# alexklwong/calibrated-backprojection-network

Hardware: AMD Instinct MI355X
Metric: depth-completion frames/sec at 352x1216 (higher is better)
Workload: dtype f32; 1 GPU; KITTI 352x1216, batch 32/GPU, fp32, full KBNet forward in HIP, random xavier weights; frames_per_gpu=32, global_batch=32, height=352, width=1216, n_ranks_seen=1, collective_backend=nccl, gathered_frames=32, launch=HIP graph replay, 2 concurrent sub-batch branch(es)

## Files before the change

calibrated-backprojection-network_amd/_lib.py:

```python

from __future__ import annotations

import ctypes as C
import os

import torch

HERE = os.path.dirname(os.path.abspath(__file__))
LIB_PATH = os.environ.get("KBN_LIB_PATH") or os.path.join(HERE, "libkbnet_hip.so")

KBN_OK = 0
KBN_ERR_INVALID_ARGUMENT, KBN_ERR_UNSUPPORTED, KBN_ERR_WORKSPACE, KBN_ERR_LAUNCH = -1, -2, -3, -4
KBN_SRC_TENSOR, KBN_SRC_COORDS, KBN_SRC_XYZ, KBN_SRC_PAIR = 0, 1, 2, 3
KBN_ACT_ELU, KBN_ACT_SIGMOID = 1, 2
KBN_RESIZE_NONE, KBN_RESIZE_NEAREST = 0, 1
KBN_MAX_SRC = 3
ABI_VERSION = 7


class KbnError(RuntimeError):
    pass


class ConvSrc(C.Structure):
    _fields_ = [
        ("kind", C.c_int),
        ("channels", C.c_int),
        ("data", C.c_void_p),
        ("batch_stride", C.c_longlong),
        ("src_height", C.c_int),
        ("src_width", C.c_int),
        ("aux_channels", C.c_int),
# ... 58 lines not shown
    "kbn_depth_head_forward": (_I, [_P, _P, _P, _P, _I, _I, _I, _I, _F, _F, _P]),
    "kbn_conv_head_forward": (_I, [_P, _L, _P, _P, _P, _P, _I, _I, _I, _I, _I, _F, _F, _F, _P]),
    "kbn_conv_tail_packed_weight_bytes": (C.c_size_t, [_I]),
    "kbn_conv_tail_pack_weight": (_I, [_P, _P, _I, _P]),
    "kbn_conv_tail_forward": (_I, [_P, _L, _P, _P, _P, _P, _I, _I, _I, _I, _I, _F, _F, _F, _P]),
    "kbn_conv_tail_forward_pair": (_I, [_P, _L, _P, _P, _P, _P, _P, _I, _I, _I, _I, _I, _F, _F, _F, _P]),
    "kbn_absmax_frames": (_I, [_P, _L, _I, _L, _P, _P]),
    "kbn_conv3x3_split_packed_weight_bytes": (C.c_size_t, [_I, _I, _I]),
    "kbn_conv3x3_split_pack_weight": (_I, [_P, _P, _I, _I, _I, _P]),
    "kbn_conv3x3_split_forward": (_I, [C.POINTER(ConvSrc), _I, _P, _P, _L, _I, _I, _I, _I, _I, _I, _I, _F, _P, _P, _L, _P, _P]),
    "kbn_conv3x3_split_forward_ksplit": (_I, [C.POINTER(ConvSrc), _I, _P, _P, _L, _I, _I, _I, _I, _I, _I, _I, _F, _P, _I, _P, _P]),
    "kbn_conv1x1s2_split_packed_weight_bytes": (C.c_size_t, [_I, _I, _I]),
    "kbn_conv1x1s2_split_pack_weight": (_I, [_P, _P, _I, _I, _I, _P]),
    "kbn_conv1x1s2_split_forward": (_I, [C.POINTER(ConvSrc), _I, _P, _P, _L, _P, _L, _I, _I, _I, _I, _I, _I, _F, _P, _P]),
    "kbn_kb_xyz_s2_forward": (_I, [_P, _L, _I, _I, _I, _P, _P, _I, _F, _P, _L, _I, _P]),
    "kbn_png_info": (_I, [_P, C.c_size_t, _P, _P, _P, _P]),
    "kbn_png_decode": (_I, [_P, C.c_size_t, _P, C.c_size_t]),
    "kbn_png_decode_batch": (_I, [_P, _P, _P, _P, _I, _I, _P]),
    "kbn_depth_to_u16_forward": (_I, [_P, _P, _L, _P]),
    "kbn_png_encode_gray16_bound": (C.c_size_t, [_I, _I]),
    "kbn_png_encode_gray16": (_I, [_P, _I, _I, _P, C.c_size_t, _P, _I]),
    "kbn_unpack_frames_forward": (_I, [_P, _P, _P, _P, _I, _I, _I, _I, _I, _I, _I, _P]),
}

_lib = None


def load():
    global _lib
    if _lib is not None:
# ... 31 lines not shown
```

calibrated-backprojection-network_amd/csrc/abi.hip:

```cpp
#include <stdlib.h>
#include <string.h>

#include "kbn_common.h"

namespace kbn {

KnobValue g_knobs[KNOB_COUNT];

static const char* const kKnobNames[KNOB_COUNT] = {
    "KBN_DEBUG", "KBN_FORCE_MW", "KBN_FORCE_TWB", "KBN_EPI_LDS", "KBN_NO_WINO",
    "KBN_NO_UP2X9", "KBN_NO_UP2X3", "KBN_WINO_RT",
    "KBN_NO_KB_PAIR", "KBN_NO_KB_DEPTH_FUSION", "KBN_PAIR_CAND", "KBN_S2D_DEBUG", "KBN_AUTOTUNE",
    "KBN_NO_HEAD_FUSION", "KBN_NO_SPLIT", "KBN_NO_OVERLAP", "KBN_NO_PAIR", "KBN_NO_PAIR_MID", "KBN_NO_PAIR_ENC",
    "KBN_NO_PAIR_TAIL", "KBN_NO_DEPTH_FRONT_FUSION", "KBN_FP16_ONE_TERM", "KBN_DEPTH_FRONT_FUSION", "KBN_NO_FRONT_NEXT"};

void tune_reload_env();

static void load_knobs() {
    for (int k = 0; k < KNOB_COUNT; ++k) {
        const char* v = getenv(kKnobNames[k]);
        g_knobs[k].set = (v && *v) ? 1 : 0;
        int val = 0;
        if (v && *v) {
            char* end = nullptr;
            const long parsed = strtol(v, &end, 10);
            val = (end == v) ? 1 : (int)parsed;
        }
        g_knobs[k].value = val;
    }
// ... 51 lines not shown
```

calibrated-backprojection-network_amd/csrc/conv_split.hip:

```cpp
#include "conv_common.h"

#ifndef KBN_SPLIT_STRAIGHT
#define KBN_SPLIT_STRAIGHT 1
#endif
#ifndef KBN_SPLIT_PRIO
#define KBN_SPLIT_PRIO 0
#endif

namespace kbn {

typedef _Float16 sph8 __attribute__((ext_vector_type(8)));
typedef _Float16 sph2 __attribute__((ext_vector_type(2)));
typedef float spf16 __attribute__((ext_vector_type(16)));
typedef float spf4 __attribute__((ext_vector_type(4)));
typedef _Float16 sph4 __attribute__((ext_vector_type(4)));

constexpr int SP_TW = 32, SP_CK = 16, SP_MB = 4, SP_TH = 16, SP_THREADS = 512;
constexpr int SP_WEXP = 13;

template <int MODE>
struct SpGeom {
    static constexpr bool UP = MODE == 1, S2 = MODE == 2;
    static constexpr int TH = S2 ? 8 : SP_TH;
    static constexpr int ROWS = UP ? TH / 2 + 2 : (S2 ? 2 * TH + 1 : TH + 2);
// ... 25 lines not shown
    unsigned* out_amax;
    const _Float16* pair_src;
    long long pair_src_bstride;
    const float* pair_src_scale;
    _Float16* pair_out;
    long long pair_out_bstride;
    float* pair_out_scale;
    const float* l1;
    int tp_x0, tp_tilesY, tp_nblocks;
    int sub0;
    const float* xyz;
    long long xyz_bstride;
    const float* wxyz;
    int ksplit;
    long long ks_stride;
};

__device__ __forceinline__ void sp_split8(const float (&v)[8], float prescale, sph8& h1, sph8& h2) {
    const float prescale_hi = prescale * 2048.f;
#pragma unroll
    for (int k = 0; k < 8; k += 2) {
        const f32x2 a = {v[k], v[k + 1]};
        const sph2 c1 = __builtin_convertvector(a * prescale, sph2);
        const f32x2 f = {(float)c1[0], (float)c1[1]};
        const f32x2 hi = a * prescale_hi;
        const f32x2 r = {__builtin_fmaf(f[0], -2048.f, hi[0]), __builtin_fmaf(f[1], -2048.f, hi[1])};
        const sph2 c2 = __builtin_convertvector(r, sph2);
        h1[k] = c1[0]; h1[k + 1] = c1[1];
        h2[k] = c2[0]; h2[k + 1] = c2[1];
    }
// ... 157 lines not shown
    const bool vec = !((reinterpret_cast<uintptr_t>(x) & 15) || (batch_stride & 3));
    const int blocks = (int)std::min<long long>(std::max(1, 2048 / n), (per_frame + 4095) / 4096);
    if (vec) hipLaunchKernelGGL(absmax_frames_kernel<true>, dim3(blocks, n), dim3(256), 0, stream, x, batch_stride, per_frame, slots);
    else hipLaunchKernelGGL(absmax_frames_kernel<false>, dim3(blocks, n), dim3(256), 0, stream, x, batch_stride, per_frame, slots);
    KBN_CHECK_LAUNCH();
    return KBN_OK;
}

template <int N, int NBX>
__device__ __forceinline__ void sp_wait_b(f32x4 (&b)[NBX][2]) {
    static_assert(NBX == 1 || NBX == 2, "one or two 32-filter blocks per wave");
    if constexpr (NBX == 2) asm volatile("s_waitcnt vmcnt(%4)" : "+v"(b[0][0]), "+v"(b[0][1]), "+v"(b[1][0]), "+v"(b[1][1]) : "n"(N));
    else asm volatile("s_waitcnt vmcnt(%2)" : "+v"(b[0][0]), "+v"(b[0][1]) : "n"(N));
}

template <int MODE, int RG, bool APART, bool BLDS, int NBW = 2, bool PIN0 = false, bool POUT = false, bool MIXED = false, bool ONE = false, bool KSPLIT = false>
__global__ __launch_bounds__(SP_THREADS, 1) void conv3x3_split_kernel(const SplitConvParams p) {
    static_assert(!MIXED || (MODE == 0 && BLDS), "transposed tiles: the concat kernel");
    extern __shared__ __attribute__((aligned(16))) unsigned char smem[];
    if (!MIXED || (int)blockIdx.x < p.nblocks) {
        constexpr bool TP = false;
        const int block = blockIdx.x, nblocks = p.nblocks, tilesX = p.tilesX, tilesY = p.tilesY;
#include "conv_split_body.inc"
    } else if constexpr (MIXED) {
        constexpr bool TP = true;
        const int block = (int)blockIdx.x - p.nblocks, nblocks = p.tp_nblocks, tilesX = 1, tilesY = p.tp_tilesY;
#include "conv_split_body.inc"
    }
}

constexpr int UF_NT = 32, UF_ITEMS = 16;
// ... 1243 lines not shown
                              void* pair_out, long long pair_out_batch_stride, float* pair_out_scale, kbn_stream_t stream) {
    return conv3x3_split_impl(srcs, n_src, packed_weight, out, out_batch_stride, n, out_channels, height, width, mode, act_exponent,
                              apply_activation, negative_slope, out_absmax, pair_out, pair_out_batch_stride, pair_out_scale, 1, nullptr, stream);
}

int kbn_conv3x3_split_forward_ksplit(const kbn_conv_src* srcs, int n_src, const void* packed_weight, float* out,
                                     long long out_batch_stride, int n, int out_channels, int height, int width, int mode,
                                     int act_exponent, int apply_activation, float negative_slope, unsigned* out_absmax,
                                     int ksplit, float* workspace, kbn_stream_t stream) {
    if (ksplit < 1) return KBN_ERR_INVALID_ARGUMENT;
    return conv3x3_split_impl(srcs, n_src, packed_weight, out, out_batch_stride, n, out_channels, height, width, mode, act_exponent,
                              apply_activation, negative_slope, out_absmax, nullptr, 0, nullptr, ksplit, workspace, stream);
}


static size_t c1_panel_bytes(int out_channels, int cin) {
    return (size_t)kbn::ceil_div(out_channels, 128) * (128 * 4 + (size_t)(cin / kbn::SP_CK) * (2 * 2 * 128 * 16));
}

size_t kbn_conv1x1s2_split_packed_weight_bytes(int out_channels, int tensor_channels, int has_xyz) {
    if (out_channels < 1 || tensor_channels < 1 || (tensor_channels % kbn::SP_CK) != 0) return 0;
    return c1_panel_bytes(out_channels, tensor_channels) + (has_xyz ? (size_t)out_channels * 3 * 4 : 0);
}

int kbn_conv1x1s2_split_pack_weight(const float* weight, void* packed, int out_channels, int in_channels, int xyz_offset,
                                    kbn_stream_t stream) {
    using namespace kbn;
    const bool has_xyz = xyz_offset >= 0;
    const int cin = in_channels - (has_xyz ? 3 : 0);
    if (!weight || !packed || (has_xyz && xyz_offset > cin) || kbn_conv1x1s2_split_packed_weight_bytes(out_channels, cin, has_xyz) == 0)
// ... 84 lines not shown
```

calibrated-backprojection-network_amd/csrc/conv_split_body.inc:

```
    static_assert(APART, "the two small terms share the scale 2^11 and an accumulator of their own");
    static_assert(!(PIN0 || POUT) || (MODE == 0 && BLDS) || (MODE == 2 && !BLDS), "pair tensors: the concat kernel and the stride-2 kernel");
    using G = SpGeom<MODE>;
    constexpr bool UP = G::UP, S2 = G::S2;
    constexpr int NB = NBW, FG = 8 / RG;
    constexpr int NT = 32 * NB * FG, NPIX = G::NPIX, PR = G::PR, COLS = TP ? 18 : G::COLS;
    static_assert(!TP || NPIX == 34 * 18, "the transposed region has the staged tile's size");
    constexpr int MB = G::TH / RG;
    static_assert(MB == 2 || MB == 4, "groups per chunk must be even (ping-pong A fragments)");
    constexpr int B_TAP = 2 * 2 * NT * 16;
    asm volatile("s_setreg_imm32_b32 hwreg(HW_REG_MODE, 6, 2), 0");
    const int tid = threadIdx.x, lane = tid & 63;
    const int wave = __builtin_amdgcn_readfirstlane(tid >> 6);
    const int rg = wave % RG, fg = wave / RG;
    const int lm = lane & 31, g = lane >> 5;
    int bid = xcd_remap(block, nblocks);
    int ks = 0;
    if constexpr (KSPLIT) { ks = bid % p.ksplit; bid /= p.ksplit; }
    const int nt = bid % p.nTilesN;
    bid /= p.nTilesN;
    const int tx = bid % tilesX;
    bid /= tilesX;
    const int ty = bid % tilesY;
    const int n = bid / tilesY;
    const int oy0 = ty * (TP ? 2 * G::TH : G::TH), ox0 = TP ? p.tp_x0 : tx * SP_TW;
// ... 394 lines not shown
                        *reinterpret_cast<spu4*>(k0 + oph + o) = g2;
                    }
                }
            }
        if (p.out_amax) absmax_commit(p.out_amax + n, amax);
        return;
    }
    const long long oplane = (long long)H * W;
    float* outn = p.out + (long long)n * p.out_bstride + (KSPLIT ? (long long)ks * p.ks_stride : 0);
    const bool vec4 = p.vec4 != 0;
#pragma unroll
    for (int nb = 0; nb < NB; ++nb) {
        const int oc = nt * NT + fg * 32 * NB + nb * 32 + lm;
        const float inv = p.inv_scale[oc] * unscale;
        if (oc >= p.OC) continue;
#pragma unroll
        for (int mb = 0; mb < MB; ++mb) {
            const int Yb = oy0 + (TP ? 2 : 1) * (MB * rg + mb);
            if (Yb >= H) continue;
#pragma unroll
            for (int q4 = 0; q4 < 4; ++q4) {
                const int Y = TP ? Yb + (q4 >> 1) : Yb;
                const int X = TP ? ox0 + 8 * (q4 & 1) + 4 * g : ox0 + 8 * q4 + 4 * g;
                if (X >= W || Y >= H) continue;
                float* o = outn + (long long)oc * oplane + (long long)Y * W + X - 8 * q4;
                f32x4 v;
#pragma unroll
                for (int j = 0; j < 4; ++j) {
                    const float t = __builtin_fmaf(lo[mb][nb][q4 * 4 + j], 0.00048828125f, acc[mb][nb][q4 * 4 + j]) * inv;
                    v[j] = t > 0.f ? t : t * slope;
                }
                if (vec4) {
                    *reinterpret_cast<f32x4*>(o + 8 * q4) = v;
                    amax = sp_amax4(amax, v);
                } else {
#pragma unroll
                    for (int j = 0; j < 4; ++j)
                        if (X + j < W) { o[8 * q4 + j] = v[j]; amax = fmaxf(amax, fin_abs(v[j])); }
                }
            }
        }
    }
    if (!KSPLIT && p.out_amax) absmax_commit(p.out_amax + n, amax);
```

calibrated-backprojection-network_amd/csrc/kbn_common.h:

```cpp
#pragma once

#include <hip/hip_runtime.h>
#include <stdint.h>

#include <atomic>

#include "../../include/kbnet_hip.h"

#define KBN_CHECK_LAUNCH()                                   \
    do {                                                     \
        hipError_t e__ = hipGetLastError();                  \
        if (e__ != hipSuccess) return KBN_ERR_LAUNCH;        \
    } while (0)

namespace kbn {

typedef float f32x4 __attribute__((ext_vector_type(4)));
typedef float f32x2 __attribute__((ext_vector_type(2)));

__host__ __device__ inline int ceil_div(int a, int b) { return (a + b - 1) / b; }
__host__ __device__ inline int round_up(int a, int b) { return ceil_div(a, b) * b; }

__device__ __forceinline__ float leaky_relu(float v, float slope) { return v > 0.f ? v : v * slope; }
__device__ __forceinline__ float fin_abs(float v) { const float a = fabsf(v); return a < __builtin_inff() ? a : 0.f; }
// ... 34 lines not shown
    std::atomic<unsigned long long>& word = once.done[(dev >> 6) & 3];
    if (word.load(std::memory_order_relaxed) & bit) return KBN_OK;
    if (hipFuncSetAttribute(kernel, hipFuncAttributeMaxDynamicSharedMemorySize, bytes) != hipSuccess)
        return KBN_ERR_LAUNCH;
    word.fetch_or(bit, std::memory_order_relaxed);
    return KBN_OK;
}
int device_cu_count();

enum Knob {
    KNOB_DEBUG, KNOB_FORCE_MW, KNOB_FORCE_TWB, KNOB_EPI_LDS, KNOB_NO_WINO,
    KNOB_NO_UP2X9, KNOB_NO_UP2X3, KNOB_WINO_RT,
    KNOB_NO_KB_PAIR, KNOB_NO_KB_DEPTH_FUSION, KNOB_PAIR_CAND, KNOB_S2D_DEBUG, KNOB_AUTOTUNE,
    KNOB_NO_HEAD_FUSION, KNOB_NO_SPLIT,
    KNOB_NO_OVERLAP, KNOB_NO_PAIR, KNOB_NO_PAIR_MID, KNOB_NO_PAIR_ENC, KNOB_NO_PAIR_TAIL, KNOB_NO_DEPTH_FRONT_FUSION,
    KNOB_FP16_ONE_TERM, KNOB_DEPTH_FRONT_FUSION, KNOB_NO_FRONT_NEXT, KNOB_COUNT
};
struct KnobValue { int set, value; };
extern KnobValue g_knobs[KNOB_COUNT];
inline int knob(Knob k) { return g_knobs[k].value; }
inline bool knob_set(Knob k) { return g_knobs[k].set != 0; }

__device__ __forceinline__ int xcd_remap(int bid, int nblocks) {
    const int NX = 8;
    int xcd = bid % NX, idx = bid / NX;
    int q = nblocks / NX, r = nblocks % NX;
    int start = (xcd < r) ? xcd * (q + 1) : r * (q + 1) + (xcd - r) * q;
    return start + idx;
}

__device__ __forceinline__ int nearest_src_index(int dst, int in_size, int out_size) {
// ... 14 lines not shown
```

calibrated-backprojection-network_amd/modules.py:

```python

from __future__ import annotations

import os
from typing import List, Optional

import torch

from . import _lib, ops
from ._lib import KbnError
from .config import KBNetConfig


def activation_func(activation_fn: str):
    if "linear" in activation_fn:
        return None
    if "leaky_relu" in activation_fn:
        return torch.nn.LeakyReLU(negative_slope=0.20, inplace=True)
    if "relu" in activation_fn:
        return torch.nn.ReLU()
    if "elu" in activation_fn:
        return torch.nn.ELU()
    if "sigmoid" in activation_fn:
        return torch.nn.Sigmoid()
    raise ValueError("Unsupported activation function: {}".format(activation_fn))
# ... 46 lines not shown
        self._args = None

    def get(self, weight: torch.Tensor, stride: int, up2x: bool = False) -> torch.Tensor:
        key = (weight.data_ptr(), weight._version, weight.device, stride, up2x)
        if key != self._key:
            if up2x == "split":
                self._packed = ops.pack_conv3x3_split_weight(weight, out=self._packed, stride=stride)
            elif up2x == "split_up":
                self._packed = ops.pack_conv3x3_split_weight(weight, out=self._packed, folded_up2x=True)
            elif up2x == "split_up_t":
                self._packed = ops.pack_conv3x3_split_weight(weight, out=self._packed, folded_up2x=True, transposed=True)
            elif up2x == "up2x_t":
                self._packed = ops.pack_upconv2x_weight(weight, out=self._packed, transposed=True)
            elif isinstance(up2x, tuple) and up2x[0] == "split_1x1s2":
                self._packed = ops.pack_conv1x1s2_split_weight(weight, up2x[1], out=self._packed)
            else:
                self._packed = (ops.pack_upconv2x_weight(weight, out=self._packed) if up2x
                                else ops.pack_conv_weight(weight, stride, out=self._packed))
            self._key = key
            self._args = (stride, up2x)
        return self._packed

    def refresh(self, weight: torch.Tensor):
        if self._packed is not None:
            self.get(weight, *self._args)


class _PackedTail:

    def __init__(self):
# ... 80 lines not shown
            raise ValueError("normalisation layers are not part of the KBNet inference path")
        if kernel_size not in (1, 3) or stride not in (1, 2):
            raise ValueError("HIP conv supports kernel_size in {1,3} and stride in {1,2}")
        self.conv = torch.nn.Conv2d(in_channels, out_channels, kernel_size=kernel_size, stride=stride,
                                    padding=kernel_size // 2, bias=False)
        _init_weight(self.conv.weight, weight_initializer)
        self.activation_func = activation_func
        self.kernel_size, self.stride = kernel_size, stride
        self.in_channels, self.out_channels = in_channels, out_channels
        self._slope = _slope(activation_func)
        self._post = _post(activation_func)
        self._packed = _PackedWeight()
        self._packed_split = _PackedWeight()
        self._packed_split_up = _PackedWeight()
        self._packed_split_1x1 = _PackedWeight()
        self.split_fused_min_filters = 192
        self.split = True
        self.split_narrow_up = True

    @staticmethod
    def _with_slots(srcs, n, dev, stats):
        for s in srcs:
            if s.kind == _lib.KBN_SRC_TENSOR and (not s.absmax or (stats is not None and not stats.usable(s.absmax))):
                if stats is None:
                    stats = ops.ActStats(n, dev, capacity=len(srcs))
                slot = stats.measure(s._keep[0])
                s.absmax = slot.data_ptr()
                s._keep = (s._keep[0], slot)
        return srcs

# ... 5 lines not shown
                and self.out_channels >= self.split_fused_min_filters and self.in_channels == ci + 3 + cf)

    def run_split_fused(self, image, fused, xyz, n, h, w, out, amax_image=None, amax_fused=None, out_absmax=None, stats=None):
        ci, cf = image.shape[1], (0 if fused is None else fused.shape[1])
        if not self.split_fused_qualifies(ci, cf):
            return None
        if isinstance(image, ops.PairTensor):
            if image.sub is None or fused is None:
                return None
            image, amax_image = image.sub, image.absmax
        srcs = [ops.tensor_src(image, "image", amax_image)] + ([] if fused is None else [ops.tensor_src(fused, "fused", amax_fused)])
        srcs = self._with_slots(srcs, n, image.device, stats)
        packed = self._packed_split_1x1.get(self.conv.weight, 2, up2x=("split_1x1s2", ci))
        return ops.conv1x1s2_split(srcs, packed, xyz, n, self.out_channels, h, w, out, negative_slope=self._slope,
                                   out_absmax=out_absmax)

    def packed(self):
        return self._packed.get(self.conv.weight, self.stride)

    def run(self, srcs, n, in_h, in_w, out=None, resize=False, out_absmax=None, stats=None):
        cin = sum(s.channels for s in srcs)
        if cin != self.in_channels:
            raise KbnError(f"expected {self.in_channels} input channels in total, got {cin}")
        oh, ow = -(-in_h // self.stride), -(-in_w // self.stride)
        if self._post is not None:
            if not resize:
                res = self.run_split(srcs, n, oh, ow, out=out, out_absmax=out_absmax, stats=stats)
                if res is not None:
                    return res
            if out is None:
# ... 181 lines not shown

    def run(self, srcs, n, h, w, out=None, out_absmax=None, stats=None):
        convs = list(self.conv_block)
        x = None
        for i, conv in enumerate(convs):
            last = i == len(convs) - 1
            x = conv.run(srcs if i == 0 else [ops.tensor_src(x, "x")], n, h, w, out=out if last else None,
                         out_absmax=out_absmax if last else None, stats=stats)
        return x

    def forward(self, x):
        return self.conv_block(x)


class CalibratedBackprojectionBlock(torch.nn.Module):

    def __init__(self, in_channels_image, in_channels_depth, in_channels_fused, n_filter_image=48,
                 n_filter_depth=16, n_filter_fused=48, n_convolution_image=1, n_convolution_depth=1,
                 n_convolution_fused=1, weight_initializer="kaiming_uniform",
                 activation_func=torch.nn.LeakyReLU(negative_slope=0.10, inplace=True)):
        super().__init__()
        self.stacked = n_convolution_image != 1 or n_convolution_depth != 1
        self.conv_image = VGGNetBlock(in_channels_image, n_filter_image, n_convolution_image, 2,
                                      weight_initializer, activation_func)
        self.conv_depth = VGGNetBlock(in_channels_depth + 3, n_filter_depth, n_convolution_depth, 2,
                                      weight_initializer, activation_func)
        self.proj_depth = Conv2d(in_channels_depth, 1, kernel_size=1, stride=1,
                                 weight_initializer=weight_initializer, activation_func=activation_func)
        self.conv_fused = Conv2d(in_channels_fused + 3, n_filter_fused, kernel_size=1, stride=2,
                                 weight_initializer=weight_initializer, activation_func=activation_func)
        self.n_filter_image, self.n_filter_depth, self.n_filter_fused = n_filter_image, n_filter_depth, n_filter_fused
        self.split_image = n_filter_image >= 96
        self.split_fused = True
        self._slope = _slope(activation_func)
        self.layerwise = self._slope is None

    def run(self, image, depth, coordinates, fused, out_image=None, out_depth=None, out_fused=None,
            amax_image=None, amax_fused=None, out_amax_image=None, out_amax_skip=None, stats=None, need_image=True,
            pair_image_out=False, fused_done=False):
        pair_in = isinstance(image, ops.PairTensor)
        if (pair_in or pair_image_out) and not (self.conv_image.conv_block[0].split and self.split_image and self.split_fused
                                                and coordinates.dim() == 3 and stats is not None
                                                and not self.stacked and not self.layerwise):
            return None
        n, ci, h, w = image.shape
        cd, cf = depth.shape[1], (0 if fused is None else fused.shape[1])
        want = (self.conv_image.conv_block[0].in_channels, self.conv_depth.conv_block[0].in_channels - 3,
                self.conv_fused.in_channels - 3 - self.conv_image.conv_block[0].in_channels)
        if (ci, cd, cf) != want:
            raise KbnError(f"KB block built for (image, depth, fused) channels {want}, got {(ci, cd, cf)}")
        if self.stacked or self.layerwise:
            return self._run_stacked(image, depth, coordinates, fused, out_image, out_depth, out_fused, out_amax_image,
                                     out_amax_skip, stats, need_image)
        oh, ow = (h + 1) // 2, (w + 1) // 2
# ... 13 lines not shown
                amax_image = image.absmax
            elif amax_image is None or (stats is not None and not stats.usable(amax_image.data_ptr())):
                stats = stats if stats is not None else ops.ActStats(n, dev, capacity=3)
                amax_image = stats.measure(image)
            branch = _SideBranch(dev)
            isrc = ops.pair_src(image, "image") if pair_in else ops.tensor_src(image, "image", amax_image)
            res = True if not need_image else ci_conv.run_split([isrc], n, oh, ow, out=out_image, out_absmax=out_amax_image, stats=stats,
                                                                pair_out=pair_image_out)
            if res is None and (pair_in or pair_image_out):
                return None
            if pair_image_out and need_image:
                out_image = res
            if res is not None:
                with branch:
                    self._depth_and_fused(image, depth, fused, kinv, n, h, w, oh, ow, out_depth, out_fused, ci, cf,
                                          amax_image, amax_fused, out_amax_skip, stats, skip_fused=fused_done)
                return out_image, out_depth, out_fused
        return ops.kb_block(image, depth, coords, kinv, fused,
                            self.conv_image.conv_block[0].packed(), self.conv_depth.conv_block[0].packed(),
                            self.proj_depth.conv.weight, self.conv_fused.packed(),
                            self.n_filter_image, self.n_filter_depth, self.n_filter_fused,
                            out_image, out_depth, out_fused, self._slope, absmax_image=out_amax_image,
                            absmax_depth=out_amax_skip, absmax_fused=out_amax_skip)

    def _run_stacked(self, image, depth, coordinates, fused, out_image, out_depth, out_fused, out_amax_image, out_amax_skip, stats,
                     need_image=True):
        n, _, h, w = image.shape
        oh, ow = (h + 1) // 2, (w + 1) // 2
        dev = image.device
        mk = lambda c: torch.empty((n, c, oh, ow), device=dev, dtype=torch.float32)
        out_image = mk(self.n_filter_image) if out_image is None else out_image
# ... 6 lines not shown
        if need_image:
            self.conv_image.run([ops.tensor_src(image, "image")], n, h, w, out=out_image, out_absmax=out_amax_image, stats=stats)
        csrc = ops.tensor_src(coordinates, "coordinates") if dense else ops.coords_src(coordinates)
        self.conv_depth.run([ops.tensor_src(depth, "depth"), csrc], n, h, w, out=out_depth, out_absmax=out_amax_skip, stats=stats)
        if self.proj_depth._post is not None:
            z = self.proj_depth.run([ops.tensor_src(depth, "depth")], n, h, w)
            xyz = ops.tensor_src(ops.scale_planes(coordinates if dense else ops.camera_coordinates(coordinates, h, w), z), "xyz")
        else:
            xyz = (ops.xyz_src(depth, self.proj_depth.conv.weight, None, coordinates=coordinates) if dense
                   else ops.xyz_src(depth, self.proj_depth.conv.weight, coordinates))
        srcs = [ops.tensor_src(image, "image"), xyz] + ([] if fused is None else [ops.tensor_src(fused, "fused")])
        self.conv_fused.run(srcs, n, h, w, out=out_fused, out_absmax=out_amax_skip, stats=stats)
        return out_image, out_depth, out_fused

    def _depth_and_fused(self, image, depth, fused, kinv, n, h, w, oh, ow, out_depth, out_fused, ci, cf, amax_image, amax_fused,
                         out_amax_skip, stats, skip_fused=False):
        self.conv_depth.conv_block[0].run([ops.tensor_src(depth, "depth"), ops.coords_src(kinv)], n, h, w, out=out_depth,
                                          out_absmax=out_amax_skip)
        if skip_fused:
            return
        if (self.split_fused and (fused is None or _dense(fused)) and self.proj_depth._slope is not None
                and self.conv_fused.split_fused_qualifies(ci, cf)):
            xyz = ops.kb_xyz_s2(depth, self.proj_depth.conv.weight, kinv, self.proj_depth._slope)
            if self.conv_fused.run_split_fused(image, fused, xyz, n, oh, ow, out_fused, amax_image, amax_fused,
                                               out_absmax=out_amax_skip, stats=stats) is not None:
                return
        if isinstance(image, ops.PairTensor):
            image = image.float()
        srcs = [ops.tensor_src(image, "image"), ops.xyz_src(depth, self.proj_depth.conv.weight, kinv)]
        if fused is not None:
            srcs.append(ops.tensor_src(fused, "fused"))
        self.conv_fused.run(srcs, n, h, w, out=out_fused, out_absmax=out_amax_skip)

# ... 281 lines not shown
                fused_done = level == 1 and next_done is not None
                if fused_done:
                    skip, a_skip = next_done
                else:
                    skip = torch.empty((n, ff[level] + fd[level], oh, ow), device=dev, dtype=torch.float32)
                out_fused, out_depth = skip[:, :ff[level]], skip[:, ff[level]:]
                unused = self.skip_unused_image and level == 3 and 4 not in self.resolutions_backprojection
                want_pair = self.pair_chain and 1 <= level < 3 and (level + 1) in self.resolutions_backprojection
                if want_pair and self._image_splitk(level + 1, oh, ow):
                    want_pair = False
                res = None
                if want_pair or isinstance(conv_image, ops.PairTensor):
                    res = blk.run(conv_image, conv_depth, kinv, conv_fused, None, out_depth, out_fused,
                                  amax_image=amax_image, amax_fused=amax_skip if conv_fused is not None else None,
                                  out_amax_image=a_img, out_amax_skip=a_skip, stats=stats, need_image=not unused,
                                  pair_image_out=want_pair, fused_done=fused_done)
                if res is None:
                    if isinstance(conv_image, ops.PairTensor):
                        conv_image, amax_image = conv_image.float(), None
                    res = blk.run(
                        conv_image, conv_depth, kinv, conv_fused, None, out_depth, out_fused,
                        amax_image=amax_image if level > 0 else None, amax_fused=amax_skip if conv_fused is not None else None,
                        out_amax_image=a_img, out_amax_skip=a_skip, stats=stats, need_image=not unused, fused_done=fused_done)
                conv_image, conv_depth, conv_fused = res
                amax_image = a_img
            else:
                src, a_src = (conv_fused, amax_skip) if conv_fused is not None else (conv_image, amax_image if level > 0 else None)
                skip = torch.empty((n, fi[level] + fd[level], oh, ow), device=dev, dtype=torch.float32)
                ci_blk = getattr(self, f"conv{level + 1}_image")
                cd_blk = getattr(self, f"conv{level + 1}_depth")
                branch = _SideBranch(dev)
                conv_image = ci_blk.run([ops.tensor_src(src, "image", a_src)], n, h, w, out=skip[:, :fi[level]], out_absmax=a_skip,
                                        stats=stats)
                with branch:
                    conv_depth = cd_blk.run([ops.tensor_src(conv_depth, "depth", amax_skip)], n, h, w, out=skip[:, fi[level]:],
                                            out_absmax=a_skip, stats=stats)
                conv_fused = None
                amax_image = a_skip
            amax_skip = a_skip
            skips.append(skip)
            amax_skips.append(a_skip)
            h, w = oh, ow
        oh, ow = (h + 1) // 2, (w + 1) // 2
        amax_latent = stats.new()
        if 4 in self.resolutions_backprojection:
            if 3 not in self.resolutions_backprojection:
                raise AttributeError("'KBNetEncoder' object has no attribute 'calibrated_backprojection4'")
            blk = self.calibrated_backprojection4
            if isinstance(conv_image, ops.PairTensor):
                conv_image, amax_image = conv_image.float(), None
            latent = torch.empty((n, blk.n_filter_fused + blk.n_filter_depth, oh, ow), device=dev, dtype=torch.float32)
            blk.run(conv_image, conv_depth, kinv1_get(), conv_fused, None, latent[:, blk.n_filter_fused:], latent[:, :blk.n_filter_fused],
                    amax_image=amax_image, amax_fused=amax_skip if conv_fused is not None else None, out_amax_image=stats.new(),
                    out_amax_skip=amax_latent, stats=stats, need_image=not self.skip_unused_image)
            return latent, skips, amax_latent, amax_skips
        latent = torch.empty((n, fi[4] + fd[4], oh, ow), device=dev, dtype=torch.float32)
        src, a_src = (conv_fused, amax_skip) if conv_fused is not None else (conv_image, amax_image)
        branch = _SideBranch(dev)
        self.conv5_image.run([ops.tensor_src(src, "image", a_src)], n, h, w, out=latent[:, :fi[4]],
                             out_absmax=amax_latent, stats=stats)
        with branch:
            self.conv5_depth.run([ops.tensor_src(conv_depth, "depth", amax_skip)], n, h, w, out=latent[:, fi[4]:],
                                 out_absmax=amax_latent, stats=stats)
        return latent, skips, amax_latent, amax_skips


class MultiScaleDecoder(torch.nn.Module):

    pair_chain = _KnobSwitch("KBN_NO_PAIR")
# ... 285 lines not shown

    def capture(self, image, sparse_depth, validity_map_depth, intrinsics, branches=None, tune=True, outputs=1, split_graphs=False):
        return GraphedForward(self, image, sparse_depth, validity_map_depth, intrinsics, branches, tune, outputs, split_graphs)

    def weight_state(self):
        return [(p.data_ptr(), p._version) for p in self.parameters()]

    def refresh_packed(self):
        for m in self.modules():
            for sub in m.modules():
                if isinstance(sub, Conv2d):
                    sub._packed.refresh(sub.conv.weight)
                    sub._packed_split.refresh(sub.conv.weight)
                    sub._packed_split_up.refresh(sub.conv.weight)
                    sub._packed_split_1x1.refresh(sub.conv.weight)
                elif isinstance(sub, UpConv2d):
                    sub._packed_up2x.refresh(sub.conv.conv.weight)
                elif isinstance(sub, TransposeConv2d):
                    sub._packed_up2x.refresh(sub.deconv.weight)
                    sub._packed_split_up.refresh(sub.deconv.weight)
                elif isinstance(sub, MultiScaleDecoder):
                    sub._packed_tail.refresh()
                elif isinstance(sub, KBNetEncoder):
                    sub._packed_front.refresh()
                    sub._packed_front_next.refresh()
                    sub._packed_depth_front.refresh()
                    sub._packed_s2d_front.refresh()

    def modules(self):
        return (self.sparse_to_dense_pool, self.encoder, self.decoder)
# ... 41 lines not shown
```

calibrated-backprojection-network_amd/ops.py:

```python

from __future__ import annotations

import contextlib
import ctypes as C
import functools
from typing import List, Optional, Sequence

import torch

from . import _lib
from ._lib import ConvSrc, KbnError, check


def _stream() -> int:
    return torch.cuda.current_stream().cuda_stream


def _on_tensor_device(fn):
    @functools.wraps(fn)
    def wrapper(*args, **kwargs):
        idx = None
        for a in list(args) + list(kwargs.values()):
            if isinstance(a, torch.Tensor) and a.is_cuda:
                if idx is None:
# ... 817 lines not shown
                     lambda: lib.kbn_conv1x1s2_split_forward(arr, len(srcs), packed_weight.data_ptr(), xptr, xbs, optr, obs, n,
                                                             out_channels, height, width, max(-60, min(60, int(act_exponent))),
                                                             0 if negative_slope is None else 1,
                                                             0.0 if negative_slope is None else float(negative_slope),
                                                             _slot_ptr(out_absmax, n), _stream()), executed=executed, pipe="fp16",
                     nbytes=4.0 * n * height * width * (cin + (3 if xyz is not None else 0) + out_channels))
    if status == _lib.KBN_ERR_UNSUPPORTED:
        if PROFILE is not None:
            PROFILE.pop()
        return None
    check(status, "kbn_conv1x1s2_split_forward")
    return out


@_on_tensor_device
def pack_kb1_front_weight(w_conv0: torch.Tensor, w_conv_image: torch.Tensor, w_conv_fused: torch.Tensor,
                          out: Optional[torch.Tensor] = None) -> Optional[torch.Tensor]:
    lib = _lib.load()
    w0, wi, wf = (w.detach().contiguous() for w in (w_conv0, w_conv_image, w_conv_fused))
    for w, nm in ((w0, "w_conv0"), (wi, "w_conv_image"), (wf, "w_conv_fused")):
        _require(w, nm, 4)
    f0, c = w0.shape[0], w0.shape[1]
    fi = wi.shape[0]
    if tuple(w0.shape[2:]) != (3, 3) or tuple(wi.shape) != (fi, f0, 3, 3) or tuple(wf.shape) != (fi, f0 + 3, 1, 1):
        return None
    nbytes = lib.kbn_kb1_front_packed_weight_bytes(c, f0, fi)
    if nbytes == 0:
        return None
    packed = out if _reusable(out, nbytes // 4, w0) else torch.empty(nbytes // 4, device=w0.device, dtype=torch.float32)
    check(lib.kbn_kb1_front_pack_weight(w0.data_ptr(), wi.data_ptr(), wf.data_ptr(), packed.data_ptr(), c, f0, fi, _stream()),
# ... 305 lines not shown
```

include/kbnet_hip.h:

```cpp
#ifndef KBNET_HIP_H
#define KBNET_HIP_H

#include <stddef.h>

#ifdef __cplusplus
extern "C" {
#endif

#define KBN_ABI_VERSION 7

typedef void* kbn_stream_t;

typedef enum kbn_status {
    KBN_OK = 0,
    KBN_ERR_INVALID_ARGUMENT = -1,
    KBN_ERR_UNSUPPORTED = -2,
    KBN_ERR_WORKSPACE = -3,
    KBN_ERR_LAUNCH = -4
} kbn_status;

int kbn_version(void);
const char* kbn_status_string(int status);

void kbn_reload_env(void);
// ... 93 lines not shown
                                     long long out_batch_stride, int n, int out_channels, int height, int width, int mode,
                                     int act_exponent, int apply_activation, float negative_slope, unsigned* out_absmax,
                                     int ksplit, float* workspace, kbn_stream_t stream);

size_t kbn_conv1x1s2_split_packed_weight_bytes(int out_channels, int tensor_channels, int has_xyz);
int kbn_conv1x1s2_split_pack_weight(const float* weight, void* packed, int out_channels, int in_channels, int xyz_offset,
                                    kbn_stream_t stream);
int kbn_conv1x1s2_split_forward(const kbn_conv_src* srcs, int n_src, const void* packed_weight, const float* xyz,
                                long long xyz_batch_stride, float* out, long long out_batch_stride, int n, int out_channels,
                                int height, int width, int act_exponent, int apply_activation, float negative_slope,
                                unsigned* out_absmax, kbn_stream_t stream);
int kbn_kb_xyz_s2_forward(const float* depth, long long depth_batch_stride, int depth_channels, int height, int width,
                          const float* proj_weight, const float* kinv, int apply_activation, float negative_slope, float* xyz,
                          long long xyz_batch_stride, int n, kbn_stream_t stream);


int kbn_conv2d_query(int n, int out_channels, int in_channels, int kernel_size, int stride,
                     int in_height, int in_width, int resize, int* info);

int kbn_kb_block_forward(const float* image, long long image_batch_stride, const float* depth,
                         long long depth_batch_stride, const float* coordinates, const float* kinv,
                         const float* fused, long long fused_batch_stride,
                         const float* packed_w_image, const float* packed_w_depth,
                         const float* proj_weight, const float* packed_w_fused, float* out_image,
                         long long out_image_batch_stride, float* out_depth,
                         long long out_depth_batch_stride, float* out_fused,
                         long long out_fused_batch_stride, int n, int height, int width,
                         int channels_image, int channels_depth, int channels_fused,
                         int filters_image, int filters_depth, int filters_fused,
                         float negative_slope, unsigned* out_image_absmax, unsigned* out_depth_absmax,
// ... 98 lines not shown
```

Baseline: 2961 frames/s.

## Route depth-branch stride-2 conv through split fp16 kernel with analytic coordinate term

Adds a stride-2 3x3 split-precision convolution for the depth branch of the calibrated backprojection blocks. The three camera-coordinate input channels are not materialised. Their contribution is computed analytically in the epilogue from kinv and precomputed per-filter weight sums, with an exact per-tap fallback at image borders. This is meant to move the depth conv off the generic fp32 path onto the faster split-fp16 matrix path and to avoid the coordinate channel reads. The cost is extra epilogue arithmetic and a new packed-weight format, and the new path can be disabled with a knob.

```diff
diff --git a/calibrated-backprojection-network_amd/_lib.py b/calibrated-backprojection-network_amd/_lib.py
--- a/calibrated-backprojection-network_amd/_lib.py
+++ b/calibrated-backprojection-network_amd/_lib.py
@@ -15,7 +15,7 @@
 KBN_ACT_ELU, KBN_ACT_SIGMOID = 1, 2
 KBN_RESIZE_NONE, KBN_RESIZE_NEAREST = 0, 1
 KBN_MAX_SRC = 3
-ABI_VERSION = 7
+ABI_VERSION = 8
 
 
 class KbnError(RuntimeError):
@@ -104,6 +104,9 @@
     "kbn_conv1x1s2_split_pack_weight": (_I, [_P, _P, _I, _I, _I, _P]),
     "kbn_conv1x1s2_split_forward": (_I, [C.POINTER(ConvSrc), _I, _P, _P, _L, _P, _L, _I, _I, _I, _I, _I, _I, _F, _P, _P]),
     "kbn_kb_xyz_s2_forward": (_I, [_P, _L, _I, _I, _I, _P, _P, _I, _F, _P, _L, _I, _P]),
+    "kbn_conv3x3s2_coords_split_packed_weight_bytes": (C.c_size_t, [_I, _I]),
+    "kbn_conv3x3s2_coords_split_pack_weight": (_I, [_P, _P, _I, _I, _P]),
+    "kbn_conv3x3s2_coords_split_forward": (_I, [C.POINTER(ConvSrc), _I, _P, _P, _P, _L, _I, _I, _I, _I, _I, _F, _P, _P]),
     "kbn_png_info": (_I, [_P, C.c_size_t, _P, _P, _P, _P]),
     "kbn_png_decode": (_I, [_P, C.c_size_t, _P, C.c_size_t]),
     "kbn_png_decode_batch": (_I, [_P, _P, _P, _P, _I, _I, _P]),
diff --git a/calibrated-backprojection-network_amd/csrc/abi.hip b/calibrated-backprojection-network_amd/csrc/abi.hip
--- a/calibrated-backprojection-network_amd/csrc/abi.hip
+++ b/calibrated-backprojection-network_amd/csrc/abi.hip
@@ -12,7 +12,8 @@
     "KBN_NO_UP2X9", "KBN_NO_UP2X3", "KBN_WINO_RT",
     "KBN_NO_KB_PAIR", "KBN_NO_KB_DEPTH_FUSION", "KBN_PAIR_CAND", "KBN_S2D_DEBUG", "KBN_AUTOTUNE",
     "KBN_NO_HEAD_FUSION", "KBN_NO_SPLIT", "KBN_NO_OVERLAP", "KBN_NO_PAIR", "KBN_NO_PAIR_MID", "KBN_NO_PAIR_ENC",
-    "KBN_NO_PAIR_TAIL", "KBN_NO_DEPTH_FRONT_FUSION", "KBN_FP16_ONE_TERM", "KBN_DEPTH_FRONT_FUSION", "KBN_NO_FRONT_NEXT"};
+    "KBN_NO_PAIR_TAIL", "KBN_NO_DEPTH_FRONT_FUSION", "KBN_FP16_ONE_TERM", "KBN_DEPTH_FRONT_FUSION", "KBN_NO_FRONT_NEXT",
+    "KBN_NO_SPLIT_DEPTH"};
 
 void tune_reload_env();
 
diff --git a/calibrated-backprojection-network_amd/csrc/conv_split.hip b/calibrated-backprojection-network_amd/csrc/conv_split.hip
--- a/calibrated-backprojection-network_amd/csrc/conv_split.hip
+++ b/calibrated-backprojection-network_amd/csrc/conv_split.hip
@@ -63,6 +63,8 @@
     const float* wxyz;
     int ksplit;
     long long ks_stride;
+    const float* kinv;
+    const float* ctab;
 };
 
 __device__ __forceinline__ void sp_split8(const float (&v)[8], float prescale, sph8& h1, sph8& h2) {
@@ -250,7 +252,45 @@
     else asm volatile("s_waitcnt vmcnt(%2)" : "+v"(b[0][0]), "+v"(b[0][1]) : "n"(N));
 }
 
-template <int MODE, int RG, bool APART, bool BLDS, int NBW = 2, bool PIN0 = false, bool POUT = false, bool MIXED = false, bool ONE = false, bool KSPLIT = false>
+constexpr int SC_TAB = 36;
+__device__ __forceinline__ float sc_coord_term(const float (&k)[9], const float (&S)[3], float cst, const float* __restrict__ raw,
+                                               int Yo, int Xo, int sH, int sW) {
+    const int Yc = 2 * Yo, Xc = 2 * Xo;
+    float c;
+    if (Yc >= 1 && Yc + 1 < sH && Xc >= 1 && Xc + 1 < sW) {
+        c = cst;
+#pragma unroll
+        for (int j = 0; j < 3; ++j) c += (__builtin_fmaf(k[3 * j + 1], (float)Yc, k[3 * j] * (float)Xc) + k[3 * j + 2]) * S[j];
+    } else {
+        c = 0.f;
+        for (int j = 0; j < 3; ++j)
+            for (int t = 0; t < 9; ++t) {
+                const int Yt = Yc + t / 3 - 1, Xt = Xc + t % 3 - 1;
+                if (Yt >= 0 && Yt < sH && Xt >= 0 && Xt < sW)
+                    c += (__builtin_fmaf(k[3 * j + 1], (float)Yt, k[3 * j] * (float)Xt) + k[3 * j + 2]) * raw[j * 9 + t];
+            }
+    }
+    return c;
+}
+__global__ void coords_tab_kernel(const float* __restrict__ w, float* __restrict__ tab, int OC, int cin_total) {
+    const int f = blockIdx.x * blockDim.x + threadIdx.x;
+    if (f >= OC) return;
+    float* t = tab + (long long)f * SC_TAB;
+    for (int j = 0; j < 3; ++j) {
+        const float* wj = w + ((long long)f * cin_total + cin_total - 3 + j) * 9;
+        float s0 = 0.f, sx = 0.f, sy = 0.f;
+        for (int q = 0; q < 9; ++q) {
+            s0 += wj[q];
+            sx += wj[q] * (float)(q % 3 - 1);
+            sy += wj[q] * (float)(q / 3 - 1);
+            t[9 + j * 9 + q] = wj[q];
+        }
+        t[j] = s0; t[3 + j] = sx; t[6 + j] = sy;
+    }
+}
+
+template <int MODE, int RG, bool APART, bool BLDS, int NBW = 2, bool PIN0 = false, bool POUT = false, bool MIXED = false, bool ONE = false, bool KSPLIT = false,
+          bool COORDS = false>
 __global__ __launch_bounds__(SP_THREADS, 1) void conv3x3_split_kernel(const SplitConvParams p) {
     static_assert(!MIXED || (MODE == 0 && BLDS), "transposed tiles: the concat kernel");
     extern __shared__ __attribute__((aligned(16))) unsigned char smem[];
@@ -1524,6 +1564,83 @@
 }
 
 
+static int sc_nt(int out_channels) { return out_channels <= 64 ? 64 : 128; }
+static size_t sc_panel_bytes(int out_channels, int cin) {
+    const int nt = sc_nt(out_channels), tiles = kbn::ceil_div(out_channels, nt);
+    return (size_t)tiles * nt * 4 + (size_t)tiles * (cin / kbn::SP_CK) * (9 * 2 * 2 * nt * 16);
+}
+
+size_t kbn_conv3x3s2_coords_split_packed_weight_bytes(int out_channels, int tensor_channels) {
+    if (out_channels < 1 || tensor_channels < 1 || (tensor_channels % kbn::SP_CK) != 0) return 0;
+    return sc_panel_bytes(out_channels, tensor_channels) + (size_t)out_channels * kbn::SC_TAB * 4;
+}
+
+int kbn_conv3x3s2_coords_split_pack_weight(const float* weight, void* packed, int out_channels, int in_channels, kbn_stream_t stream) {
+    using namespace kbn;
+    const int cin = in_channels - 3;
+    if (!weight || !packed || kbn_conv3x3s2_coords_split_packed_weight_bytes(out_channels, cin) == 0) return KBN_ERR_INVALID_ARGUMENT;
+    const int nt = sc_nt(out_channels), ocpad = ceil_div(out_channels, nt) * nt;
+    float* inv = static_cast<float*>(packed);
+    _Float16* wp = reinterpret_cast<_Float16*>(inv + ocpad);
+    const long long total = (long long)((sc_panel_bytes(out_channels, cin) - (size_t)ocpad * 4) / 2);
+    hipLaunchKernelGGL(split_scale_kernel, dim3(ocpad), dim3(256), 0, (hipStream_t)stream, weight, inv, out_channels, in_channels * 9);
+    hipLaunchKernelGGL(pack_split_kernel, dim3((unsigned)((total + 255) / 256)), dim3(256), 0, (hipStream_t)stream, weight, inv, wp,
+                       out_channels, cin, cin / SP_CK, nt, total, 9, cin, 3);
+    hipLaunchKernelGGL(coords_tab_kernel, dim3(ceil_div(out_channels, 64)), dim3(64), 0, (hipStream_t)stream, weight,
+                       reinterpret_cast<float*>(static_cast<unsigned char*>(packed) + sc_panel_bytes(out_channels, cin)), out_channels,
+                       in_channels);
+    KBN_CHECK_LAUNCH();
+    return KBN_OK;
+}
+
+int kbn_conv3x3s2_coords_split_forward(const kbn_conv_src* srcs, int n_src, const void* packed_weight, const float* kinv, float* out,
+                                       long long out_batch_stride, int n, int out_channels, int height, int width, int apply_activation,
+                                       float negative_slope, unsigned* out_absmax, kbn_stream_t stream) {
+    using namespace kbn;
+    if (!srcs || n_src != 1 || !packed_weight || !kinv || !out || n < 1 || out_channels < 1 || height < 1 || width < 1)
+        return KBN_ERR_INVALID_ARGUMENT;
+    if (knob(KNOB_NO_SPLIT) || knob(KNOB_NO_SPLIT_DEPTH)) return KBN_ERR_UNSUPPORTED;
+    const kbn_conv_src& a = srcs[0];
+    if (a.kind != KBN_SRC_TENSOR || !a.data || a.channels < 1 || (a.channels % SP_CK) != 0) return KBN_ERR_UNSUPPORTED;
+    if (ceil_div(a.src_height, 2) != height || ceil_div(a.src_width, 2) != width) return KBN_ERR_INVALID_ARGUMENT;
+    if ((long long)a.src_height * a.src_width > 0x1fffffffLL) return KBN_ERR_UNSUPPORTED;
+    SplitConvParams p{};
+    p.src[0] = p.src[1] = a.data;
+    p.src_bstride[0] = p.src_bstride[1] = a.batch_stride;
+    p.srcC[0] = a.channels; p.srcC[1] = 0;
+    p.nsrc = 1;
+    p.sH = a.src_height; p.sW = a.src_width;
+    p.amax[0] = a.absmax; p.amax[1] = nullptr;
+    p.out_amax = out_absmax;
+    const int cin = a.channels, nt = sc_nt(out_channels);
+    p.nTilesN = ceil_div(out_channels, nt);
+    p.inv_scale = static_cast<const float*>(packed_weight);
+    p.wp = reinterpret_cast<const _Float16*>(p.inv_scale + p.nTilesN * nt);
+    p.ctab = reinterpret_cast<const float*>(static_cast<const unsigned char*>(packed_weight) + sc_panel_bytes(out_channels, cin));
+    p.kinv = kinv;
+    p.out = out; p.out_bstride = out_batch_stride;
+    p.N = n; p.OC = out_channels; p.Cin = cin; p.H = height; p.W = width;
+    p.tilesX = ceil_div(width, SP_TW); p.tilesY = ceil_div(height, SpGeom<2>::TH);
+    const long long blocks = (long long)p.tilesX * p.tilesY * n * p.nTilesN;
+    if (blocks > 0x7fffffffLL) return KBN_ERR_UNSUPPORTED;
+    p.nblocks = (int)blocks;
+    p.act = apply_activation ? 1 : 0; p.slope = negative_slope;
+    p.prescale = ldexpf(1.f, -6); p.unscale = ldexpf(1.f, 6);
+    p.vec4 = ((width & 3) || (reinterpret_cast<uintptr_t>(out) & 15) || (out_batch_stride & 3)) ? 0 : 1;
+    p.ksplit = 1;
+    static DeviceOnce o64, o128;
+    auto launch = [&](auto kern, DeviceOnce& once) -> int {
+        if (int rc = set_max_dynamic_lds(once, reinterpret_cast<const void*>(kern), 160 * 1024)) return rc;
+        hipLaunchKernelGGL(kern, dim3(p.nblocks), dim3(SP_THREADS), SpGeom<2>::LDS, (hipStream_t)stream, p);
+        return KBN_OK;
+    };
+    const int rc = nt == 64 ? launch(conv3x3_split_kernel<2, 4, true, false, 1, false, false, false, false, false, true>, o64)
+                            : launch(conv3x3_split_kernel<2, 2, true, false, 1, false, false, false, false, false, true>, o128);
+    if (rc != KBN_OK) return rc;
+    KBN_CHECK_LAUNCH();
+    return KBN_OK;
+}
+
 static size_t c1_panel_bytes(int out_channels, int cin) {
     return (size_t)kbn::ceil_div(out_channels, 128) * (128 * 4 + (size_t)(cin / kbn::SP_CK) * (2 * 2 * 128 * 16));
 }
diff --git a/calibrated-backprojection-network_amd/csrc/conv_split_body.inc b/calibrated-backprojection-network_amd/csrc/conv_split_body.inc
--- a/calibrated-backprojection-network_amd/csrc/conv_split_body.inc
+++ b/calibrated-backprojection-network_amd/csrc/conv_split_body.inc
@@ -1,4 +1,5 @@
     static_assert(APART, "the two small terms share the scale 2^11 and an accumulator of their own");
+    static_assert(!COORDS || (MODE == 2 && !PIN0 && !POUT && !KSPLIT && !ONE), "coordinate channels: the stride-2 kernel, fp32 in and out");
     static_assert(!(PIN0 || POUT) || (MODE == 0 && BLDS) || (MODE == 2 && !BLDS), "pair tensors: the concat kernel and the stride-2 kernel");
     using G = SpGeom<MODE>;
     constexpr bool UP = G::UP, S2 = G::S2;
@@ -432,6 +433,17 @@
         const int oc = nt * NT + fg * 32 * NB + nb * 32 + lm;
         const float inv = p.inv_scale[oc] * unscale;
         if (oc >= p.OC) continue;
+        float ck[9], cS[3], ccst = 0.f;
+        const float* craw = nullptr;
+        if constexpr (COORDS) {
+            const float* ki = p.kinv + (long long)n * 9;
+#pragma unroll
+            for (int i = 0; i < 9; ++i) ck[i] = ki[i];
+            const float* sm = p.ctab + (long long)oc * SC_TAB;
+#pragma unroll
+            for (int j = 0; j < 3; ++j) { cS[j] = sm[j]; ccst += ck[3 * j] * sm[3 + j] + ck[3 * j + 1] * sm[6 + j]; }
+            craw = sm + 9;
+        }
 #pragma unroll
         for (int mb = 0; mb < MB; ++mb) {
             const int Yb = oy0 + (TP ? 2 : 1) * (MB * rg + mb);
@@ -445,7 +457,8 @@
                 f32x4 v;
 #pragma unroll
                 for (int j = 0; j < 4; ++j) {
-                    const float t = __builtin_fmaf(lo[mb][nb][q4 * 4 + j], 0.00048828125f, acc[mb][nb][q4 * 4 + j]) * inv;
+                    float t = __builtin_fmaf(lo[mb][nb][q4 * 4 + j], 0.00048828125f, acc[mb][nb][q4 * 4 + j]) * inv;
+                    if constexpr (COORDS) t += sc_coord_term(ck, cS, ccst, craw, Y, X + j, sH, sW);
                     v[j] = t > 0.f ? t : t * slope;
                 }
                 if (vec4) {
diff --git a/calibrated-backprojection-network_amd/csrc/kbn_common.h b/calibrated-backprojection-network_amd/csrc/kbn_common.h
--- a/calibrated-backprojection-network_amd/csrc/kbn_common.h
+++ b/calibrated-backprojection-network_amd/csrc/kbn_common.h
@@ -72,7 +72,7 @@
     KNOB_NO_KB_PAIR, KNOB_NO_KB_DEPTH_FUSION, KNOB_PAIR_CAND, KNOB_S2D_DEBUG, KNOB_AUTOTUNE,
     KNOB_NO_HEAD_FUSION, KNOB_NO_SPLIT,
     KNOB_NO_OVERLAP, KNOB_NO_PAIR, KNOB_NO_PAIR_MID, KNOB_NO_PAIR_ENC, KNOB_NO_PAIR_TAIL, KNOB_NO_DEPTH_FRONT_FUSION,
-    KNOB_FP16_ONE_TERM, KNOB_DEPTH_FRONT_FUSION, KNOB_NO_FRONT_NEXT, KNOB_COUNT
+    KNOB_FP16_ONE_TERM, KNOB_DEPTH_FRONT_FUSION, KNOB_NO_FRONT_NEXT, KNOB_NO_SPLIT_DEPTH, KNOB_COUNT
 };
 struct KnobValue { int set, value; };
 extern KnobValue g_knobs[KNOB_COUNT];
diff --git a/calibrated-backprojection-network_amd/modules.py b/calibrated-backprojection-network_amd/modules.py
--- a/calibrated-backprojection-network_amd/modules.py
+++ b/calibrated-backprojection-network_amd/modules.py
@@ -84,6 +84,8 @@
                 self._packed = ops.pack_upconv2x_weight(weight, out=self._packed, transposed=True)
             elif isinstance(up2x, tuple) and up2x[0] == "split_1x1s2":
                 self._packed = ops.pack_conv1x1s2_split_weight(weight, up2x[1], out=self._packed)
+            elif up2x == "split_s2_coords":
+                self._packed = ops.pack_conv3x3s2_coords_split_weight(weight, out=self._packed)
             else:
                 self._packed = (ops.pack_upconv2x_weight(weight, out=self._packed) if up2x
                                 else ops.pack_conv_weight(weight, stride, out=self._packed))
@@ -194,6 +196,7 @@
         self._packed_split = _PackedWeight()
         self._packed_split_up = _PackedWeight()
         self._packed_split_1x1 = _PackedWeight()
+        self._packed_split_coords = _PackedWeight()
         self.split_fused_min_filters = 192
         self.split = True
         self.split_narrow_up = True
@@ -229,6 +232,16 @@
         packed = self._packed_split_1x1.get(self.conv.weight, 2, up2x=("split_1x1s2", ci))
         return ops.conv1x1s2_split(srcs, packed, xyz, n, self.out_channels, h, w, out, negative_slope=self._slope,
                                    out_absmax=out_absmax)
+
+    def run_split_coords(self, depth, kinv, n, h, w, out, amax_depth=None, out_absmax=None, stats=None):
+        cd = depth.shape[1]
+        if (not self.split or getattr(self, "latency", 0) or self.kernel_size != 3 or self.stride != 2 or self._post is not None
+                or cd % 16 or cd < 32 or self.in_channels != cd + 3 or not ops.split_enabled()):
+            return None
+        srcs = self._with_slots([ops.tensor_src(depth, "depth", amax_depth)], n, depth.device, stats)
+        packed = self._packed_split_coords.get(self.conv.weight, 2, up2x="split_s2_coords")
+        return ops.conv3x3s2_coords_split(srcs[0], packed, kinv, n, self.out_channels, h, w, out, negative_slope=self._slope,
+                                          out_absmax=out_absmax)
 
     def packed(self):
         return self._packed.get(self.conv.weight, self.stride)
@@ -440,6 +453,7 @@
 
 
 class CalibratedBackprojectionBlock(torch.nn.Module):
+    split_depth = _KnobSwitch("KBN_NO_SPLIT_DEPTH")
 
     def __init__(self, in_channels_image, in_channels_depth, in_channels_fused, n_filter_image=48,
                  n_filter_depth=16, n_filter_fused=48, n_convolution_image=1, n_convolution_depth=1,
@@ -463,7 +477,7 @@
 
     def run(self, image, depth, coordinates, fused, out_image=None, out_depth=None, out_fused=None,
             amax_image=None, amax_fused=None, out_amax_image=None, out_amax_skip=None, stats=None, need_image=True,
-            pair_image_out=False, fused_done=False):
+            pair_image_out=False, fused_done=False, amax_depth=None):
         pair_in = isinstance(image, ops.PairTensor)
         if (pair_in or pair_image_out) and not (self.conv_image.conv_block[0].split and self.split_image and self.split_fused
                                                 and coordinates.dim() == 3 and stats is not None
@@ -507,7 +521,7 @@
             if res is not None:
                 with branch:
                     self._depth_and_fused(image, depth, fused, kinv, n, h, w, oh, ow, out_depth, out_fused, ci, cf,
-                                          amax_image, amax_fused, out_amax_skip, stats, skip_fused=fused_done)
+                                          amax_image, amax_fused, out_amax_skip, stats, skip_fused=fused_done, amax_depth=amax_depth)
                 return out_image, out_depth, out_fused
         return ops.kb_block(image, depth, coords, kinv, fused,
                             self.conv_image.conv_block[0].packed(), self.conv_depth.conv_block[0].packed(),
@@ -544,9 +558,11 @@
         return out_image, out_depth, out_fused
 
     def _depth_and_fused(self, image, depth, fused, kinv, n, h, w, oh, ow, out_depth, out_fused, ci, cf, amax_image, amax_fused,
-                         out_amax_skip, stats, skip_fused=False):
-        self.conv_depth.conv_block[0].run([ops.tensor_src(depth, "depth"), ops.coords_src(kinv)], n, h, w, out=out_depth,
-                                          out_absmax=out_amax_skip)
+                         out_amax_skip, stats, skip_fused=False, amax_depth=None):
+        cd_conv = self.conv_depth.conv_block[0]
+        if not (self.split_depth and _dense(depth) and cd_conv.run_split_coords(depth, kinv, n, oh, ow, out_depth, amax_depth,
+                                                                                out_amax_skip, stats) is not None):
+            cd_conv.run([ops.tensor_src(depth, "depth"), ops.coords_src(kinv)], n, h, w, out=out_depth, out_absmax=out_amax_skip)
         if skip_fused:
             return
         if (self.split_fused and (fused is None or _dense(fused)) and self.proj_depth._slope is not None
@@ -858,14 +874,15 @@
                     res = blk.run(conv_image, conv_depth, kinv, conv_fused, None, out_depth, out_fused,
                                   amax_image=amax_image, amax_fused=amax_skip if conv_fused is not None else None,
                                   out_amax_image=a_img, out_amax_skip=a_skip, stats=stats, need_image=not unused,
-                                  pair_image_out=want_pair, fused_done=fused_done)
+                                  pair_image_out=want_pair, fused_done=fused_done, amax_depth=amax_skip)
                 if res is None:
                     if isinstance(conv_image, ops.PairTensor):
                         conv_image, amax_image = conv_image.float(), None
                     res = blk.run(
                         conv_image, conv_depth, kinv, conv_fused, None, out_depth, out_fused,
                         amax_image=amax_image if level > 0 else None, amax_fused=amax_skip if conv_fused is not None else None,
-                        out_amax_image=a_img, out_amax_skip=a_skip, stats=stats, need_image=not unused, fused_done=fused_done)
+                        out_amax_image=a_img, out_amax_skip=a_skip, stats=stats, need_image=not unused, fused_done=fused_done,
+                        amax_depth=amax_skip)
                 conv_image, conv_depth, conv_fused = res
                 amax_image = a_img
             else:
@@ -896,7 +913,7 @@
             latent = torch.empty((n, blk.n_filter_fused + blk.n_filter_depth, oh, ow), device=dev, dtype=torch.float32)
             blk.run(conv_image, conv_depth, kinv1_get(), conv_fused, None, latent[:, blk.n_filter_fused:], latent[:, :blk.n_filter_fused],
                     amax_image=amax_image, amax_fused=amax_skip if conv_fused is not None else None, out_amax_image=stats.new(),
-                    out_amax_skip=amax_latent, stats=stats, need_image=not self.skip_unused_image)
+                    out_amax_skip=amax_latent, stats=stats, need_image=not self.skip_unused_image, amax_depth=amax_skip)
             return latent, skips, amax_latent, amax_skips
         latent = torch.empty((n, fi[4] + fd[4], oh, ow), device=dev, dtype=torch.float32)
         src, a_src = (conv_fused, amax_skip) if conv_fused is not None else (conv_image, amax_image)
@@ -1212,6 +1229,7 @@
                     sub._packed_split.refresh(sub.conv.weight)
                     sub._packed_split_up.refresh(sub.conv.weight)
                     sub._packed_split_1x1.refresh(sub.conv.weight)
+                    sub._packed_split_coords.refresh(sub.conv.weight)
                 elif isinstance(sub, UpConv2d):
                     sub._packed_up2x.refresh(sub.conv.conv.weight)
                 elif isinstance(sub, TransposeConv2d):
diff --git a/calibrated-backprojection-network_amd/ops.py b/calibrated-backprojection-network_amd/ops.py
--- a/calibrated-backprojection-network_amd/ops.py
+++ b/calibrated-backprojection-network_amd/ops.py
@@ -855,6 +855,50 @@
 
 
 @_on_tensor_device
+def pack_conv3x3s2_coords_split_weight(weight: torch.Tensor, out: Optional[torch.Tensor] = None) -> torch.Tensor:
+    lib = _lib.load()
+    w = weight.detach().contiguous()
+    _require(w, "weight", 4)
+    oc, cin, kh, kw = w.shape
+    nbytes = lib.kbn_conv3x3s2_coords_split_packed_weight_bytes(oc, cin - 3) if (kh, kw) == (3, 3) else 0
+    if nbytes == 0:
+        raise KbnError(f"conv3x3s2_coords_split needs a 3x3 weight with (in_channels - 3) % 16 == 0, got {tuple(w.shape)}")
+    packed = out if _reusable(out, nbytes // 4, w) else torch.empty(nbytes // 4, device=w.device, dtype=torch.float32)
+    check(lib.kbn_conv3x3s2_coords_split_pack_weight(w.data_ptr(), packed.data_ptr(), oc, cin, _stream()),
+          "kbn_conv3x3s2_coords_split_pack_weight")
+    return packed
+
+
+def conv3x3s2_coords_split(src: ConvSrc, packed_weight: torch.Tensor, kinv: torch.Tensor, n: int, out_channels: int, height: int,
+                           width: int, out: torch.Tensor, negative_slope: Optional[float] = 0.2,
+                           out_absmax: Optional[torch.Tensor] = None):
+    lib = _lib.load()
+    _require(kinv, "kinv", 3)
+    if tuple(kinv.shape) != (n, 3, 3) or not kinv.is_contiguous():
+        raise KbnError("conv3x3s2_coords_split: kinv must be a dense N x 3 x 3")
+    arr = (ConvSrc * 1)(src)
+    optr, obs = _planes(out, "out")
+    if tuple(out.shape) != (n, out_channels, height, width):
+        raise KbnError(f"out has shape {tuple(out.shape)}, expected {(n, out_channels, height, width)}")
+    cin = src.channels
+    flops = 2.0 * n * height * width * (cin + 3) * 9 * out_channels
+    nt = 64 if out_channels <= 64 else 128
+    executed = 3 * 2.0 * n * (-(-height // 8) * 8) * (-(-width // 32) * 32) * cin * 9 * (-(-out_channels // nt) * nt)
+    status = _launch("conv_split_s2_coords", flops,
+                     lambda: lib.kbn_conv3x3s2_coords_split_forward(arr, 1, packed_weight.data_ptr(), kinv.data_ptr(), optr, obs, n,
+                                                                    out_channels, height, width, 0 if negative_slope is None else 1,
+                                                                    0.0 if negative_slope is None else float(negative_slope),
+                                                                    _slot_ptr(out_absmax, n), _stream()),
+                     executed=executed, pipe="fp16", nbytes=_src_bytes([src], n) + 4.0 * n * height * width * out_channels)
+    if status == _lib.KBN_ERR_UNSUPPORTED:
+        if PROFILE is not None:
+            PROFILE.pop()
+        return None
+    check(status, "kbn_conv3x3s2_coords_split_forward")
+    return out
+
+
+@_on_tensor_device
 def pack_kb1_front_weight(w_conv0: torch.Tensor, w_conv_image: torch.Tensor, w_conv_fused: torch.Tensor,
                           out: Optional[torch.Tensor] = None) -> Optional[torch.Tensor]:
     lib = _lib.load()
diff --git a/include/kbnet_hip.h b/include/kbnet_hip.h
--- a/include/kbnet_hip.h
+++ b/include/kbnet_hip.h
@@ -7,7 +7,7 @@
 extern "C" {
 #endif
 
-#define KBN_ABI_VERSION 7
+#define KBN_ABI_VERSION 8
 
 typedef void* kbn_stream_t;
 
@@ -131,6 +131,12 @@
                           const float* proj_weight, const float* kinv, int apply_activation, float negative_slope, float* xyz,
                           long long xyz_batch_stride, int n, kbn_stream_t stream);
 
+size_t kbn_conv3x3s2_coords_split_packed_weight_bytes(int out_channels, int tensor_channels);
+int kbn_conv3x3s2_coords_split_pack_weight(const float* weight, void* packed, int out_channels, int in_channels, kbn_stream_t stream);
+int kbn_conv3x3s2_coords_split_forward(const kbn_conv_src* srcs, int n_src, const void* packed_weight, const float* kinv, float* out,
+                                       long long out_batch_stride, int n, int out_channels, int height, int width, int apply_activation,
+                                       float negative_slope, unsigned* out_absmax, kbn_stream_t stream);
+
 
 int kbn_conv2d_query(int n, int out_channels, int in_channels, int kernel_size, int stride,
                      int in_height, int in_width, int resize, int* info);
```

After: 2972 frames/s, median of 6. About the same (+0.4%).
